# kernel-matrix-benchmarks/kernel-matrix-benchmarks

Measured on AMD Instinct MI355X. Metric: point-pair interactions/s (N*M/s) + max |err| vs scipy, D=3 Gaussian, higher is better.
Workload: dtype f32

## Files before the change

### kernel_matrix_benchmarks_amd/csrc/kmvp_api.hip

```cpp
#include "kmvp_ctx.hpp"

namespace kmvp {

Rccl g_rccl;

namespace {
thread_local std::string g_create_error;
}

int fail(kmvp_ctx* c, int code, const std::string& msg) {
  if (c) c->err = msg;
  else g_create_error = msg;
  return code;
}
const char* create_error() { return g_create_error.c_str(); }

int ensure(kmvp_ctx* c, DevBuf& b, size_t bytes) {
  if (bytes <= b.cap && b.p) return KMVP_OK;
  if (b.p) {
    HIP_TRY(c, hipFree(b.p));
    b.p = nullptr;
    b.cap = 0;
  }
  if (bytes == 0) bytes = 16;
// ... 38 lines not shown
  kmvp_ctx* c = new kmvp_ctx();
  c->device = device;
  bool ok = hipSetDevice(device) == hipSuccess &&
            hipStreamCreateWithFlags(&c->stream, hipStreamNonBlocking) == hipSuccess;
  for (int i = 0; ok && i < 5; ++i) ok = hipEventCreate(&c->ev[i]) == hipSuccess;
  if (!ok) {
    fail(nullptr, KMVP_E_DEVICE, "cannot create stream/events on the device");
    if (status) *status = KMVP_E_DEVICE;
    kmvp_destroy(c);
    return nullptr;
  }
  if (status) *status = KMVP_OK;
  return c;
}

void kmvp_destroy(kmvp_ctx* c) {
  if (!c) return;
  (void)hipSetDevice(c->device);
  if (c->stream) (void)hipStreamSynchronize(c->stream);
  if (c->comm && g_rccl.CommDestroy) g_rccl.CommDestroy(c->comm);
  for (DevBuf* b : {&c->y_raw, &c->x_raw, &c->b_raw, &c->xs, &c->rec, &c->x_scaled, &c->y_scaled,
                    &c->part, &c->partd, &c->aux, &c->sortbuf, &c->perm, &c->sums, &c->out, &c->scratch, &c->sdiag, &c->precond, &c->knn, &c->xchg, &c->kexp, &c->kshift, &c->xchgk, &c->kflag,
                    &c->sk_xs_x, &c->sk_rec_y, &c->sk_xs_y, &c->sk_rec_x, &c->sk_state, &c->km_xs, &c->km_rec, &c->km_part, &c->km_state, &c->ms_xs, &c->ms_state, &c->ms_tmp,
                    &c->cell_tperm, &c->cell_sperm, &c->cell_tgrp, &c->cell_sgrp, &c->cell_slot, &c->cell_tmeta, &c->cell_sums, &c->cell_skey, &c->cell_scentre, &c->cell_scale})
    release(*b);
  for (int i = 0; i < 5; ++i)
    if (c->ev[i]) (void)hipEventDestroy(c->ev[i]);
  if (c->stream) (void)hipStreamDestroy(c->stream);
  delete c;
}

const char* kmvp_last_error(const kmvp_ctx* c) { return c ? c->err.c_str() : create_error(); }

int kmvp_set_points(kmvp_ctx* c, const void* y, int64_t M, const void* x_or_null, int64_t N, int D,
                    int dtype, int64_t j_offset, int64_t M_total) {
  if (!c) return KMVP_E_INVALID;
  if (dtype != KMVP_F32 && dtype != KMVP_F64 && dtype != KMVP_BF16)
    return fail(c, KMVP_E_INVALID, "unknown dtype");
  if (M < 0 || N < 0 || D < 1) return fail(c, KMVP_E_INVALID, "bad shape");
  if ((M > 0 && !y) || (N > 0 && !x_or_null && N != M))
    return fail(c, KMVP_E_INVALID, "same_points (x == NULL) needs N == M");
  if (M_total < M || j_offset < 0 || j_offset + M > M_total)
    return fail(c, KMVP_E_INVALID, "shard [j_offset, j_offset+M) is outside [0, M_total)");
  HIP_TRY(c, hipSetDevice(c->device));
  const size_t es = elem_size(dtype);
  int rc;
  if ((rc = ensure(c, c->y_raw, (size_t)M * D * es))) return rc;
// ... 274 lines not shown

int kmvp_set_option(kmvp_ctx* c, const char* key, int64_t value) {
  if (!c || !key) return KMVP_E_INVALID;
  const std::string k(key);
  if (k == "feed") {
    if (value < -1 || value > 1) return fail(c, KMVP_E_INVALID, "feed must be -1 (auto), 0 or 1");
    c->opt_feed = (int)value;
  } else if (k == "targets_per_lane") {
    if (value != 0 && value != 1 && value != 2 && value != 4 && value != 8)
      return fail(c, KMVP_E_INVALID, "targets_per_lane must be 0 (auto), 1, 2, 4 or 8");
    c->opt_T = (int)value;
  } else if (k == "segments") {
    if (value < 0 || value > 65535) return fail(c, KMVP_E_INVALID, "segments out of range");
    c->opt_segments = (int)value;
  } else if (k == "fast_sqdists") {
    if (value < -1 || value > 4) return fail(c, KMVP_E_INVALID, "fast_sqdists must be -1 (auto), 0, 1, 2, 3 or 4");
    c->opt_fast = (int)value;
  } else if (k == "cellmm_shape") {
    if (value < -1 || value > 1) return fail(c, KMVP_E_INVALID, "cellmm_shape must be -1 (by size), 0 (32x32x16) or 1 (16x16x32)");
    c->opt_cellmm_shape = (int)value;
  } else if (k == "cell_fused") {
    if (value < -1 || value > 1) return fail(c, KMVP_E_INVALID, "cell_fused must be -1 (automatic), 0 (two launches) or 1 (one launch where it applies)");
    c->opt_cell_fused = (int)value;
  } else if (k == "cell_shared_build") {
    if (value < -1 || value > 1) return fail(c, KMVP_E_INVALID, "cell_shared_build must be -1 (automatic), 0 (never) or 1 (wherever a workgroup is one-cell)");
    c->opt_cell_shared_build = (int)value;
  } else if (k == "mfma_variant") {
    if (value != -1 && value != 0 && value != 1 && value != 4 && value != 5)
      return fail(c, KMVP_E_INVALID, "mfma_variant must be -1 (by kernel), 0, 1, 4 or 5");
    c->opt_mfma_variant = (int)value;
  } else if (k == "same_points_global") {
    c->opt_same_global = value != 0;
  } else if (k == "partial_shard") {
    c->opt_partial = value != 0;
  } else if (k == "fast_tiles") {
    if (value != 0 && value != 1 && value != 2 && value != 4 && value != 8)
      return fail(c, KMVP_E_INVALID, "fast_tiles must be 0 (auto), 1, 2, 4 or 8");
    c->opt_fast_tiles = (int)value;
  } else if (k == "meanshift_compact") {
    if (value < -1 || value > 1) return fail(c, KMVP_E_INVALID, "meanshift_compact must be -1 (default), 0 or 1");
    c->opt_meanshift_compact = (int)value;
  } else if (k == "chunk") {
    if (value < 8 || value > (1 << 24)) return fail(c, KMVP_E_INVALID, "chunk out of range");
    c->opt_chunk = (int)value;
  } else {
    return fail(c, KMVP_E_INVALID, "unknown option " + k);
  }
  return KMVP_OK;
}

int64_t kmvp_device_bytes(const kmvp_ctx* c) {
  if (!c) return 0;
  size_t t = 0;
  for (const DevBuf* b : {&c->y_raw, &c->x_raw, &c->b_raw, &c->xs, &c->rec, &c->x_scaled,
                          &c->y_scaled, &c->part, &c->partd, &c->aux, &c->sortbuf, &c->perm, &c->sums, &c->out, &c->scratch, &c->sdiag, &c->precond, &c->knn, &c->xchg, &c->kexp, &c->kshift, &c->xchgk, &c->kflag,
                    &c->sk_xs_x, &c->sk_rec_y, &c->sk_xs_y, &c->sk_rec_x, &c->sk_state, &c->km_xs, &c->km_rec, &c->km_part, &c->km_state, &c->ms_xs, &c->ms_state, &c->ms_tmp,
                          &c->cell_tperm, &c->cell_sperm, &c->cell_tgrp, &c->cell_sgrp, &c->cell_slot, &c->cell_tmeta, &c->cell_sums, &c->cell_skey, &c->cell_scentre, &c->cell_scale})
    t += b->cap;
  return (int64_t)t;
}
double kmvp_last_kernel_ms(const kmvp_ctx* c) { return c ? c->last_kernel_ms : 0.0; }
double kmvp_last_total_ms(const kmvp_ctx* c) { return c ? c->last_total_ms : 0.0; }
double kmvp_last_allreduce_ms(const kmvp_ctx* c) { return c ? c->last_allreduce_ms : 0.0; }
const char* kmvp_last_kernel_name(const kmvp_ctx* c) { return c ? c->last_kernel_name : ""; }
const char* kmvp_last_dispatch_note(const kmvp_ctx* c) { return c ? c->note.c_str() : ""; }

}
```

### kernel_matrix_benchmarks_amd/csrc/kmvp_cell.hpp

```cpp
#pragma once
#include <hip/hip_runtime.h>
#include <stdint.h>

#include "kmvp_fast.hpp"

namespace kmvp {

constexpr int CELL_STAGE_TILES = 4;
constexpr int CELL_A_BYTES = CELL_TILE * 32;
constexpr int CELL_TILE_BYTES = CELL_A_BYTES + CELL_TILE * 16;
constexpr int CELL_HDR_OFF = CELL_STAGE_TILES * CELL_TILE_BYTES;
constexpr int CELL_STAGE_BYTES = 8192;
static_assert(CELL_HDR_OFF + CELL_STAGE_TILES * 16 <= CELL_STAGE_BYTES, "stage image too small");
constexpr float CELL_T_MAX = 0.016f;
constexpr int CELL_MAX_GRID = 1024;

struct CellGrid {
  float lo[3];
  float h[3], inv_h[3];
  int g[3];
};

__host__ __device__ inline float cell_centre(unsigned key, int a, const CellGrid& grid) {
  return grid.lo[a] + ((float)((key >> (10 * a)) & 1023u) + 0.5f) * grid.h[a];
}

struct CellArgs {
  const float* xd;
  const float* tmeta;
  const unsigned char* img;
  double* part;
  int64_t n_slots;
  int64_t tile_base;
  int64_t m_stages;
  int64_t seg_stages;
  int segments;
  int tile_blocks;
  int chunk_stages;
};

template <int SIG, int TT>
__global__ void __launch_bounds__(BLOCK_THREADS) cell_kernel(const CellArgs a) {
  constexpr int NE = (SIG == SIG_NORM) ? 2 : 1;
  constexpr int SB = CELL_STAGE_BYTES;
  constexpr int PIECES = SB / (16 * BLOCK_THREADS);
  constexpr float LOG2E = 1.4426950408889634f;
// ... 180 lines not shown
```

### kernel_matrix_benchmarks_amd/csrc/kmvp_cell_pack.hpp

```cpp
#pragma once
#include "kmvp_cell.hpp"

namespace kmvp {

__global__ void cell_keys_kernel(const float* __restrict__ p, int64_t n, int D, CellGrid grid,
                                 unsigned* __restrict__ keys, int* __restrict__ vals) {
  const int64_t i = (int64_t)blockIdx.x * blockDim.x + threadIdx.x;
  if (i >= n) return;
  unsigned key = 0;
  for (int a = 0; a < D; ++a) {
    int c = (int)floorf((p[i * D + a] - grid.lo[a]) * grid.inv_h[a]);
    c = c < 0 ? 0 : (c >= grid.g[a] ? grid.g[a] - 1 : c);
    key |= (unsigned)c << (10 * a);
  }
  keys[i] = key;
  vals[i] = (int)i;
}

__global__ void __launch_bounds__(CELL_TILE) pack_cell_targets_kernel(
    const float* __restrict__ x, const int* __restrict__ perm, const int* __restrict__ gstart,
    const int* __restrict__ gcnt, const unsigned* __restrict__ gkey, int64_t n_groups, int D, CellGrid grid,
    float* __restrict__ xd, float* __restrict__ tmeta, int* __restrict__ slot_of) {
  const int64_t g = blockIdx.x;
  const int r = threadIdx.x;
  const int64_t gg = g < n_groups ? g : n_groups - 1;
  const unsigned key = gkey[gg];
  const bool valid = g < n_groups && r < gcnt[g];
  const int64_t idx = valid ? perm[gstart[g] + r] : 0;
  float d[4] = {0.f, 0.f, 0.f, 0.f}, c[3] = {0.f, 0.f, 0.f};
  for (int a = 0; a < D; ++a) {
    c[a] = cell_centre(key, a, grid);
    d[a] = valid ? x[idx * D + a] - c[a] : 0.f;
  }
  *reinterpret_cast<f32x4*>(xd + (g * CELL_TILE + r) * 4) = f32x4{d[0], d[1], d[2], 0.f};
  const bool empty = g >= n_groups || gcnt[g] == 0;
  if (r == 0)
    *reinterpret_cast<f32x4*>(tmeta + g * 4) = f32x4{c[0], c[1], c[2], __builtin_bit_cast(float, key | (empty ? 1u << 30 : 0u))};
  if (valid) slot_of[idx] = (int)(g * CELL_TILE + r);
// ... 62 lines not shown
```

### kernel_matrix_benchmarks_amd/csrc/kmvp_cellmm_pack.hpp

```cpp
#pragma once
#include "kmvp_cellmm.hpp"

namespace kmvp {

__global__ void __launch_bounds__(CELL_TILE) pack_cellmm_points_kernel(
    const float* __restrict__ y, const int* __restrict__ perm, const int* __restrict__ gstart,
    const int* __restrict__ gcnt, const unsigned* __restrict__ gkey, int64_t n_groups, int D, CellGrid grid,
    unsigned char* __restrict__ img) {
  const int64_t g = blockIdx.x;
  const int r = threadIdx.x;
  unsigned char* stage = img + (g / CMM_STAGE_TILES) * CMM_STAGE_BYTES;
  const int q = (int)(g % CMM_STAGE_TILES);
  const bool real_tile = g < n_groups;
  const unsigned key = real_tile ? gkey[g] : 0u;
  const bool valid = real_tile && r < gcnt[g];
  const int64_t idx = valid ? perm[gstart[g] + r] : 0;
  float e[3] = {0.f, 0.f, 0.f}, c[3] = {0.f, 0.f, 0.f};
  for (int a = 0; a < D; ++a) {
    c[a] = cell_centre(key, a, grid);
    e[a] = valid ? y[idx * D + a] - c[a] : 0.f;
  }
  const float e2 = e[0] * e[0] + e[1] * e[1] + e[2] * e[2];
  *reinterpret_cast<f32x4*>(stage + CMM_E_OFF + (q * CELL_TILE + r) * 16) =
      f32x4{2.f * e[0], 2.f * e[1], 2.f * e[2], e2 * -1.4426950408889634f};
  if (r == 0)
    *reinterpret_cast<f32x4*>(stage + CMM_HDR_OFF + q * 16) =
        f32x4{c[0], c[1], c[2], __int_as_float(real_tile ? (int)key : -1)};
}

__global__ void cellmm_absmax_kernel(const float* __restrict__ b, int64_t n, int E, int col, unsigned* __restrict__ out) {
  unsigned m = 0;
  for (int64_t i = (int64_t)blockIdx.x * blockDim.x + threadIdx.x; i < n; i += (int64_t)gridDim.x * blockDim.x) {
    const unsigned v = (unsigned)__float_as_int(b[i * E + col]) & 0x7fffffffu;
    m = v > m ? v : m;
  }
  for (int off = 32; off > 0; off >>= 1) {
    const unsigned o = (unsigned)__shfl_xor((int)m, off);
    m = o > m ? o : m;
  }
  if ((threadIdx.x & 63) == 0 && m) atomicMax(out, m);
}

__global__ void cellmm_scale_kernel(const unsigned* __restrict__ bmax_bits, int wlog2, int density,
                                    float* __restrict__ scale) {
  float bmax = density ? 1.f : __int_as_float((int)*bmax_bits);
  int ex = 0;
  if (bmax > 0.f && bmax < INFINITY) {
    int eb;
    (void)frexpf(bmax * 0.104f, &eb);
    ex = 15 - eb - wlog2;
    ex = ex < -100 ? -100 : (ex > 100 ? 100 : ex);
  }
  scale[0] = ldexpf(1.f, ex);
  scale[1] = ldexpf(1.f, -ex - 6);
}

__global__ void __launch_bounds__(CELL_TILE) pack_cellmm_signal_kernel(
    const float* __restrict__ b, int E, int col, const int* __restrict__ perm, const int* __restrict__ gstart,
    const int* __restrict__ gcnt, int64_t n_groups, const float* __restrict__ scale, unsigned char* __restrict__ img) {
  const int64_t g = blockIdx.x;
  const int r = threadIdx.x;
  unsigned char* stage = img + (g / CMM_STAGE_TILES) * CMM_STAGE_BYTES;
  const int q = (int)(g % CMM_STAGE_TILES);
  const bool valid = g < n_groups && r < gcnt[g];
  const float bj = valid ? (b ? b[(int64_t)perm[gstart[g] + r] * E + col] : 1.f) : 0.f;
  *reinterpret_cast<float*>(stage + CMM_B_OFF + (q * CELL_TILE + r) * 4) = bj * scale[0];
}

}
```

### kernel_matrix_benchmarks_amd/csrc/kmvp_ctx.hpp

```cpp
#pragma once
#include <dlfcn.h>
#include <hip/hip_runtime.h>
#include <rccl/rccl.h>
#include <stdint.h>
#include <stdlib.h>
#include <string.h>

#include <algorithm>
#include <cmath>
#include <string>
#include <vector>

#include "../../include/kmvp.h"
#include "kmvp_internal.hpp"

namespace kmvp {

enum : int { LAYOUT_LOWD = 0, LAYOUT_FAST = 1, LAYOUT_MFMA = 2, LAYOUT_CFAST = 3, LAYOUT_CELL = 4, LAYOUT_CELL64 = 5, LAYOUT_CELLMM = 6, LAYOUT_FASTMM = 7, LAYOUT_CFASTMM = 8 };

struct DevBuf {
  void* p = nullptr;
  size_t cap = 0;
};

// ... 60 lines not shown
  using DevBuf = kmvp::DevBuf;
  int device = 0;
  hipStream_t stream = nullptr;
  hipEvent_t ev[5] = {nullptr, nullptr, nullptr, nullptr, nullptr};
  std::string err;

  int dtype = -1;
  int D = 0, E = 0;
  int64_t M = 0, N = 0, j_offset = 0, m_total = 0;
  bool same_points = false;
  bool have_points = false, have_signal = false, density = false;
  bool async_product = false;
  bool diag_on = false;
  int64_t diag_n = 0;
  double diag_ridge = 0.0, diag_min = 0.0;

  DevBuf y_raw, x_raw, b_raw;
  DevBuf xs, rec;
  DevBuf partd;
  DevBuf aux;
  DevBuf sortbuf, perm;
  DevBuf x_scaled, y_scaled;
  DevBuf cell_tperm, cell_sperm, cell_tgrp, cell_sgrp, cell_slot, cell_tmeta, cell_sums, cell_skey, cell_scentre, cell_scale;
  DevBuf part, sums, out;
  DevBuf xchg;
  DevBuf kexp, kshift, xchgk;
  DevBuf kflag;
  DevBuf scratch;
  DevBuf knn;
  DevBuf sdiag;
  DevBuf precond;
  int precond_rank = 0;
  int pc_built = 0;
  int pc_used = 0;
  int pc_kernel = -1, pc_rank = 0;
  uint64_t pc_points_ver = 0, pc_diag_ver = 0;
  uint64_t diag_ver = 0;
  float last_precond_ms = 0.f;
  double pc_logdet_c = 0.0;
  DevBuf sk_xs_x, sk_rec_y, sk_xs_y, sk_rec_x, sk_state;
  uint64_t sk_points_ver = 0;
  DevBuf km_xs, km_rec, km_part, km_state;
  uint64_t km_points_ver = 0;
  DevBuf ms_xs, ms_state, ms_tmp;
  uint64_t points_ver = 0, signal_ver = 0;
  int packed_layout = -1;
  int packed_kernel = -1, packed_sig = -1, packed_T = -1;
  uint64_t packed_points_ver = 0, packed_signal_ver = 0;
  int gen_kernel = -1;
  uint64_t gen_points_ver = 0;
  int64_t out_n = 0;
  int out_e = 0;

  int opt_feed = -1, opt_T = 0, opt_segments = 0, opt_chunk = 512;
  int opt_fast = -1, opt_fast_tiles = 0;
  int opt_cellmm_shape = -1;
  int opt_cell_shared_build = -1;
  int opt_cell_fused = -1;
  int opt_mfma_variant = -1;
  int opt_meanshift_compact = -1;
  int opt_same_global = 0;
  int opt_partial = 0;
  uint64_t perm_ver = 0;
  uint64_t cell_ver = 0;
  int cell_state = 0;
  int cell_tt = 0, cell_tt_req = 0;
  float cell_lo[3] = {0.f, 0.f, 0.f}, cell_hh[3] = {1.f, 1.f, 1.f};
  int cell_g[3] = {1, 1, 1};
  int64_t cell_n_tiles = 0, cell_m_tiles = 0;
  int64_t cell_n_main = 0, cell_n_rest = 0;
  float cloud_radius2 = INFINITY;
  uint64_t centre_ver = 0;

  ncclComm_t comm = nullptr;
  int rank = 0, world = 1;
  kmvp_host_allreduce_fn host_xchg = nullptr;
  void* host_user = nullptr;
  std::vector<double> host_buf;
  bool exchanges() const { return comm != nullptr || host_xchg != nullptr; }

  int comm_count = 1;
  float last_kernel_ms = 0.f, last_total_ms = 0.f, last_allreduce_ms = 0.f;
  const char* last_kernel_name = "";
  std::string note;
};

namespace kmvp {

// ... 83 lines not shown
```

### kernel_matrix_benchmarks_amd/csrc/kmvp_plan.hpp

```cpp
#pragma once
#include <algorithm>
#include <cstdint>
#include <vector>

namespace kmvp {

constexpr int WAVES_PER_BLOCK = 4;
constexpr int CELL_TILE = 32;
constexpr int CELL_REST_TT = 2;
constexpr int STAGED_TILE = 32;
constexpr int64_t SMALL_PROBLEM_TARGETS = 32768;
constexpr int SEG_SPLIT_FROM = 16;
constexpr int64_t MAX_GRID = 0x7fffffff;

inline int64_t round_up(int64_t v, int64_t q) { return (v + q - 1) / q * q; }
inline bool small_problem(int64_t N) { return N < SMALL_PROBLEM_TARGETS; }


struct SegmentRule {
  int64_t stage_bytes;
  int cols;
  int64_t min_seg = 1;
  bool small = false;
  int64_t l2_seg_bytes = 2 << 20;
// ... 191 lines not shown
  g.main_grid = s.grid(0);
  g.rest_grid = s.grid(1);
  g.total = g.main_grid + g.rest_grid;
  g.fused = opt_fused != 0 && tt > CELL_REST_TT && s.blocks[1] > 0 && g.total <= MAX_GRID;
  return g;
}


constexpr int CELL_SHARED_TT = 8;

constexpr bool cell_shared_build(int tt, int opt) { return opt != 0 && tt >= CELL_SHARED_TT; }

inline int64_t count_one_cell_blocks(const unsigned* keys, int64_t n_main, int tt) {
  const int64_t per_block = (int64_t)tt * WAVES_PER_BLOCK;
  int64_t one = 0;
  for (int64_t t = 0; t + per_block <= n_main; t += per_block) {
    bool same = true;
    for (int w = 1; w < WAVES_PER_BLOCK; ++w) same = same && keys[t + (int64_t)w * tt] == keys[t];
    one += same ? 1 : 0;
  }
  return one;
}

}
```

### kernel_matrix_benchmarks_amd/csrc/kmvp_product.hip

```cpp
#include "kmvp_ctx.hpp"
#include <vector>
#include "kmvp_cell_pack.hpp"
#include "kmvp_cell64_pack.hpp"
#include "kmvp_cellmm_pack.hpp"
#include "kmvp_cfast_pack.hpp"
#include "kmvp_fast_pack.hpp"
#include "kmvp_fastmm_pack.hpp"
#include "kmvp_cfastmm_pack.hpp"
#include "kmvp_mfma_pack.hpp"

namespace kmvp {
namespace {

template <typename real>
hipError_t launch_lowd(int kernel, int D, int E, int sig, LowdTuning tune,
                       const LowdArgs<real>& args, dim3 grid, hipStream_t s, const char** name);
template <>
hipError_t launch_lowd<float>(int kernel, int D, int E, int sig, LowdTuning tune,
                              const LowdArgs<float>& args, dim3 grid, hipStream_t s,
                              const char** name) {
  switch (kernel) {
    case K_GAUSSIAN: return launch_lowd_gaussian_f32(D, E, sig, tune, args, grid, s, name);
    case K_ABSEXP: return launch_lowd_absexp_f32(D, E, sig, tune, args, grid, s, name);
    case K_INVDIST: return launch_lowd_invdist_f32(D, E, sig, tune, args, grid, s, name);
// ... 1109 lines not shown
  a.scale = scale;
  a.m_total = c->m_total;
  const dim3 grid((unsigned)p.grid);
  const int64_t pieces = m_stages * (CF_GROUP / 32) * (MODE ? 2 : 1) * 2 * 64;
  return run_column_blocks(
      c, key, sig, p, cb, false, online ? "cfastmm_kernel with the per-target online shift (targets != sources)" : nullptr,
      [&](int col0, int nb) {
        hipLaunchKernelGGL(pack_cfastmm_signal_kernel, dim3(blocks_for(pieces)), dim3(256), 0, c->stream,
                           (const float*)c->b_raw.p, (const float*)cb.sigma, (const int*)c->perm.p, (unsigned char*)c->rec.p,
                           M, m_stages, E, col0, nb, MODE);
      },
      [&](int nb) {
        a.NE = nb;
        a.part = (double*)c->part.p;
        hipError_t le = launch_cfastmm(kernel, MODE, TT, online, a, grid, c->stream, &c->last_kernel_name);
        if (le == hipErrorInvalidValue) return fail(c, KMVP_E_UNSUPPORTED, "no cfastmm_kernel for this kernel / tile count");
        HIP_TRY(c, le);
        return (int)KMVP_OK;
      });
}


int cell_sort(kmvp_ctx* c, const void* pts, int64_t n, const CellGrid& grid, kmvp_ctx::DevBuf& perm,
              std::vector<unsigned>& keys, kmvp_ctx::DevBuf* keys_dev = nullptr) {
  int rc;
  const int D = c->D;
  const size_t keys_bytes = (size_t)n * sizeof(unsigned);
  SortBufs b;
  if ((rc = sort_buffers(c, n, b))) return rc;
  if ((rc = ensure(c, perm, (size_t)n * sizeof(int)))) return rc;
  if (c->dtype == KMVP_F64)
    hipLaunchKernelGGL(cell64_keys_kernel, dim3(blocks_for(n)), dim3(256), 0, c->stream, (const double*)pts, n, D, grid,
                       b.keys_in, b.vals_in);
  else
    hipLaunchKernelGGL(cell_keys_kernel, dim3(blocks_for(n)), dim3(256), 0, c->stream, (const float*)pts, n, D, grid,
                       b.keys_in, b.vals_in);
  HIP_TRY(c, hipGetLastError());
  HIP_TRY(c, sort_pairs_u32(b.tmp, &b.tmp_bytes, b.keys_in, b.keys_out, b.vals_in, (int*)perm.p, n, c->stream));
  keys.resize((size_t)n);
  HIP_TRY(c, hipMemcpyAsync(keys.data(), b.keys_out, keys_bytes, hipMemcpyDeviceToHost, c->stream));
  if (keys_dev) {
    if ((rc = ensure(c, *keys_dev, keys_bytes))) return rc;
    HIP_TRY(c, hipMemcpyAsync(keys_dev->p, b.keys_out, keys_bytes, hipMemcpyDeviceToDevice, c->stream));
  }
  HIP_TRY(c, hipStreamSynchronize(c->stream));
  return KMVP_OK;
}

int upload_tiles(kmvp_ctx* c, const TileList& l, kmvp_ctx::DevBuf& grp) {
  const size_t G = l.size();
  int rc;
  if ((rc = ensure(c, grp, 3 * std::max<size_t>(G, 1) * sizeof(int)))) return rc;
  HIP_TRY(c, hipMemcpyAsync(grp.p, l.start.data(), G * sizeof(int), hipMemcpyHostToDevice, c->stream));
  HIP_TRY(c, hipMemcpyAsync((int*)grp.p + G, l.count.data(), G * sizeof(int), hipMemcpyHostToDevice, c->stream));
  HIP_TRY(c, hipMemcpyAsync((int*)grp.p + 2 * G, l.key.data(), G * sizeof(int), hipMemcpyHostToDevice, c->stream));
  HIP_TRY(c, hipStreamSynchronize(c->stream));
// ... 14 lines not shown
    if (!(cells <= CELL_MAX_GRID)) return false;
    grid.g[a] = (int)cells;
    if (half > 0.f) {
      grid.h[a] = (float)(2.0 * half / cells);
      grid.inv_h[a] = 1.f / grid.h[a];
    }
  }
  return true;
}
void cell_store_grid(kmvp_ctx* c, const CellGrid& grid) {
  for (int a = 0; a < 3; ++a) {
    c->cell_lo[a] = grid.lo[a];
    c->cell_g[a] = grid.g[a];
    c->cell_hh[a] = grid.h[a];
  }
}
void cell_load_grid(const kmvp_ctx* c, CellGrid& grid) {
  for (int a = 0; a < 3; ++a) {
    grid.lo[a] = c->cell_lo[a];
    grid.g[a] = c->cell_g[a];
    grid.h[a] = c->cell_hh[a];
    grid.inv_h[a] = 1.f / c->cell_hh[a];
  }
}

inline double cell_ps_per_tile(int TT) { return TT >= 8 ? CMM_PS_PER_TILE_MAIN : (TT >= 4 ? CMM_PS_PER_TILE_TT4 : CMM_PS_PER_TILE_REST); }

int cell_prepare(kmvp_ctx* c, int TT) {
  if (c->cell_ver == c->points_ver && c->cell_state != 0 && (c->cell_state < 0 || c->cell_tt_req == TT)) return KMVP_OK;
  c->cell_tt_req = TT;
  c->cell_ver = c->points_ver;
  c->cell_state = -1;
  const int D = c->D;
  if (D > CELL_MAX_D || !(c->cloud_radius2 < INFINITY) || c->N > 0x3fffffff || c->M > 0x3fffffff) return KMVP_OK;
  float aux[FAST_AUX_FLOATS];
  HIP_TRY(c, hipMemcpyAsync(aux, c->aux.p, sizeof(aux), hipMemcpyDeviceToHost, c->stream));
  HIP_TRY(c, hipStreamSynchronize(c->stream));
  CellGrid grid;
  if (!cell_make_grid(aux, D, (float)(std::sqrt(2.f * CELL_T_MAX / (float)D)), grid)) return KMVP_OK;
  int rc;
  std::vector<unsigned> keys;
  if ((rc = cell_sort(c, c->y_raw.p, c->M, grid, c->cell_sperm, keys))) return rc;
  const TileList sources = cell_tiles(keys.data(), c->M);
  if ((rc = upload_tiles(c, sources, c->cell_sgrp))) return rc;
  c->cell_m_tiles = (int64_t)sources.size();
  if (!c->same_points && (rc = cell_sort(c, c->x_raw.p, c->N, grid, c->cell_tperm, keys))) return rc;
  if (TT == 0) {
    double best = INFINITY;
    for (int t : {8, 4, 2}) {
      int64_t nm, nr;
      cell_split_count(keys.data(), (int64_t)keys.size(), t, &nm, &nr);
      const double cost = cell_ps_per_tile(t) * (double)nm + cell_ps_per_tile(2) * (double)nr;
      if (cost < best) {
        best = cost;
        TT = t;
      }
    }
  }
  if ((rc = upload_tiles(c, cell_tiles_split(keys.data(), (int64_t)keys.size(), TT, &c->cell_n_main, &c->cell_n_rest), c->cell_tgrp)))
    return rc;
  c->cell_n_tiles = c->cell_n_main + c->cell_n_rest;
  c->cell_tt = TT;
  cell_store_grid(c, grid);
  c->cell_state = 1;
  c->packed_layout = -1;
  return KMVP_OK;
}

double cell_padding(const kmvp_ctx* c) {
  const double t = (double)c->cell_n_tiles * CELL_TILE / (double)std::max<int64_t>(c->N, 1);
  const double s = (double)c->cell_m_tiles * CELL_TILE / (double)std::max<int64_t>(c->M, 1);
  return std::max(t, s);
}

CellSplit cell_plan(const kmvp_ctx* c, int stage_tiles, SegmentRule main) {
  return cell_split(c->N, c->cell_m_tiles, c->cell_n_main, c->cell_n_rest, c->cell_tt, c->opt_segments, stage_tiles, main);
}
double* cell_region(const kmvp_ctx* c, const CellSplit& s, int cols, int r) { return (double*)c->part.p + s.region_offset(cols, r); }
template <class Args>
void cell_args(const kmvp_ctx* c, const CellSplit& s, int cols, int r, Args& a) {
  a.part = cell_region(c, s, cols, r);
  a.n_slots = s.slots[r];
  a.tile_base = r ? c->cell_n_main : 0;
  a.seg_stages = s.seg_stages[r];
  a.segments = s.segments[r];
  a.tile_blocks = (int)s.blocks[r];
}
inline int cell_tt(const kmvp_ctx* c, int r) { return r ? CELL_REST_TT : c->cell_tt; }

int pack_cell_targets(kmvp_ctx* c, const CellGrid& grid) {
  const int64_t n_tiles = c->cell_n_tiles;
  const float* x_raw = (const float*)(c->same_points ? c->y_raw.p : c->x_raw.p);
  const int* tperm = (const int*)(c->same_points ? c->cell_sperm.p : c->cell_tperm.p);
  const int* tgrp = (const int*)c->cell_tgrp.p;
  int rc;
  if ((rc = ensure(c, c->xs, (size_t)n_tiles * CELL_TILE * 4 * sizeof(float)))) return rc;
  if ((rc = ensure(c, c->cell_tmeta, (size_t)n_tiles * 4 * sizeof(float)))) return rc;
  if ((rc = ensure(c, c->cell_slot, (size_t)c->N * sizeof(int)))) return rc;
  hipLaunchKernelGGL(pack_cell_targets_kernel, dim3((unsigned)n_tiles), dim3(CELL_TILE), 0, c->stream, x_raw, tperm,
                     tgrp, tgrp + n_tiles, (const unsigned*)(tgrp + 2 * n_tiles), n_tiles, c->D,
                     grid, (float*)c->xs.p, (float*)c->cell_tmeta.p, (int*)c->cell_slot.p);
  return KMVP_OK;
}


int run_product_cell(kmvp_ctx* c, int sig) {
  const int D = c->D;
  const int E = 1;
  const int NE = sig == SIG_NORM ? 2 : 1;
  const int64_t N = c->N;
  SegmentRule rule(CELL_STAGE_BYTES, NE);
  rule.min_seg = 4;
  const CellSplit s = cell_plan(c, CELL_STAGE_TILES, rule);
  const int64_t m_stages = s.m_stages, n_slots = s.n_slots;
  int rc;
  CellGrid grid;
  cell_load_grid(c, grid);

  const PackKey key = {LAYOUT_CELL, K_GAUSSIAN, c->cell_tt};
  const int* sgrp = (const int*)c->cell_sgrp.p;
  if (points_stale(c, key) && (rc = pack_cell_targets(c, grid))) return rc;
  if (signal_stale(c, key, sig)) {
    if ((rc = ensure(c, c->rec, (size_t)m_stages * CELL_STAGE_BYTES))) return rc;
    hipLaunchKernelGGL(pack_cell_sources_kernel, dim3((unsigned)(m_stages * CELL_STAGE_TILES)), dim3(CELL_TILE), 0,
                       c->stream, (const float*)c->y_raw.p,
                       sig == SIG_DENSITY ? (const float*)nullptr : (const float*)c->b_raw.p,
                       (const int*)c->cell_sperm.p, sgrp, sgrp + c->cell_m_tiles,
                       (const unsigned*)(sgrp + 2 * c->cell_m_tiles), c->cell_m_tiles, D, grid,
                       (unsigned char*)c->rec.p);
  }
  HIP_TRY(c, hipGetLastError());
  record_packed(c, key, sig);

  if ((rc = ensure(c, c->part, s.part_doubles(NE) * sizeof(double)))) return rc;
  CellArgs a;
  a.xd = (const float*)c->xs.p;
  a.tmeta = (const float*)c->cell_tmeta.p;
  a.img = (const unsigned char*)c->rec.p;
  a.m_stages = m_stages;
  a.chunk_stages = std::max(1, c->opt_chunk / (CELL_TILE * CELL_STAGE_TILES));
  HIP_TRY(c, mark(c, 0));
  hipError_t le = hipSuccess;
  for (int r = 0; r < 2 && le == hipSuccess; ++r)
    if (s.blocks[r] > 0) {
      cell_args(c, s, NE, r, a);
      le = launch_cell_gaussian(sig, cell_tt(c, r), a, dim3((unsigned)s.grid(r)), c->stream, &c->last_kernel_name);
    }
  if (le == hipErrorInvalidValue) return fail(c, KMVP_E_UNSUPPORTED, "fast_tiles must be 1, 2, 4 or 8");
  HIP_TRY(c, le);
  HIP_TRY(c, mark(c, 1));

  if ((rc = ensure(c, c->sums, (size_t)NE * N * sizeof(double)))) return rc;
  if ((rc = ensure(c, c->cell_sums, (size_t)NE * n_slots * sizeof(double)))) return rc;
  for (int r = 0; r < 2; ++r)
    if (s.blocks[r] > 0)
      hipLaunchKernelGGL(reduce_region_kernel, dim3(blocks_for((int64_t)NE * s.slots[r])), dim3(256), 0, c->stream,
                         (const double*)cell_region(c, s, NE, r), (double*)c->cell_sums.p, s.slots[r], NE, s.segments[r], n_slots,
                         r ? s.slots[0] : (int64_t)0);
  hipLaunchKernelGGL(gather_cells_kernel, dim3(blocks_for((int64_t)NE * N)), dim3(256), 0, c->stream,
                     (const double*)c->cell_sums.p, (const int*)c->cell_slot.p, (double*)c->sums.p, N, n_slots, NE);
  HIP_TRY(c, hipGetLastError());
  return finish_product(c, (int64_t)NE * N, N, N, E, sig);
}


int cellmm_wlog2(const kmvp_ctx* c) {
  double arg = 0.0;
  for (int a = 0; a < c->D; ++a) arg += (double)c->cell_hh[a] * ((double)c->cell_g[a] * c->cell_hh[a]);
  return (int)std::ceil(arg * 1.4426950408889634);
}

int run_product_cellmm(kmvp_ctx* c, int sig) {
  const int D = c->D;
  const int E = sig == SIG_DENSITY ? 1 : c->E;
  const int NE = sig == SIG_NORM ? E + 1 : E;
  const int64_t N = c->N;
  const int TT = c->cell_tt;
  SegmentRule rule(CMM_STAGE_BYTES, 1);
  rule.min_seg = 2;
  rule.l2_seg_bytes = 3 << 20;
  rule.target_blocks = 7168;
  const CellSplit s = cell_plan(c, CMM_STAGE_TILES, rule);
  const int64_t m_stages = s.m_stages, n_slots = s.n_slots;
  int rc;
  CellGrid grid;
  cell_load_grid(c, grid);

  const PackKey key = {LAYOUT_CELLMM, K_GAUSSIAN, TT};
  const int image_sig = NE > 1 ? -1 : sig;
  const bool sig_stale = signal_stale(c, key, image_sig);
  const int* sgrp = (const int*)c->cell_sgrp.p;
  if ((rc = ensure(c, c->cell_scale, 64))) return rc;
  float* scale = (float*)c->cell_scale.p;
  unsigned* bmax = (unsigned*)c->cell_scale.p + 4;
  HIP_TRY(c, mark(c, 0));
  if (points_stale(c, key)) {
    if ((rc = pack_cell_targets(c, grid))) return rc;
    if ((rc = ensure(c, c->rec, (size_t)m_stages * CMM_STAGE_BYTES))) return rc;
    hipLaunchKernelGGL(pack_cellmm_points_kernel, dim3((unsigned)(m_stages * CMM_STAGE_TILES)), dim3(CELL_TILE), 0,
                       c->stream, (const float*)c->y_raw.p, (const int*)c->cell_sperm.p, sgrp, sgrp + c->cell_m_tiles,
                       (const unsigned*)(sgrp + 2 * c->cell_m_tiles), c->cell_m_tiles, D, grid, (unsigned char*)c->rec.p);
    HIP_TRY(c, hipGetLastError());
  }
  record_packed(c, key, image_sig);

  if ((rc = ensure(c, c->part, s.part_doubles(1) * sizeof(double)))) return rc;
  if ((rc = ensure(c, c->sums, (size_t)NE * N * sizeof(double)))) return rc;
  if ((rc = ensure(c, c->cell_sums, (size_t)NE * n_slots * sizeof(double)))) return rc;
  const int shape = c->opt_cellmm_shape >= 0 ? c->opt_cellmm_shape : ((TT >= 8 && c->N >= 500000 && c->M >= 100000) ? 1 : 0);
  FusedCellGrid fg = fused_cell_grid(s, TT, c->opt_cell_fused);
  if (shape != 1) fg.fused = false;
  CellmmArgs a;
  a.xd = (const float*)c->xs.p;
  a.tmeta = (const float*)c->cell_tmeta.p;
  a.img = (const unsigned char*)c->rec.p;
  a.scale = scale;
  a.m_stages = m_stages;
  a.shared_build = cell_shared_build(TT, c->opt_cell_shared_build) ? 1 : 0;
  if (NE == 1 && !sig_stale) HIP_TRY(c, mark(c, 0));
  for (int col = 0; col < NE; ++col) {
    if (sig_stale) {
      const float* b = (sig == SIG_DENSITY || col == E) ? (const float*)nullptr : (const float*)c->b_raw.p;
      HIP_TRY(c, hipMemsetAsync(bmax, 0, sizeof(unsigned), c->stream));
      if (b)
        hipLaunchKernelGGL(cellmm_absmax_kernel, dim3((unsigned)std::min<int64_t>(1024, (c->M + 255) / 256)), dim3(256), 0,
                           c->stream, b, c->M, E, col, bmax);
      hipLaunchKernelGGL(cellmm_scale_kernel, dim3(1), dim3(1), 0, c->stream, (const unsigned*)bmax, cellmm_wlog2(c),
                         b ? 0 : 1, scale);
      hipLaunchKernelGGL(pack_cellmm_signal_kernel, dim3((unsigned)(m_stages * CMM_STAGE_TILES)), dim3(CELL_TILE), 0,
                         c->stream, b, E, col, (const int*)c->cell_sperm.p, sgrp, sgrp + c->cell_m_tiles, c->cell_m_tiles,
                         (const float*)scale, (unsigned char*)c->rec.p);
      HIP_TRY(c, hipGetLastError());
      if (NE == 1) HIP_TRY(c, mark(c, 0));
    }
    hipError_t le = hipSuccess;
    if (fg.fused) {
      CellmmArgs ar = a;
      cell_args(c, s, 1, 0, a);
      cell_args(c, s, 1, 1, ar);
      le = launch_cellmm16_fused(TT, a, ar, fg.main_grid, fg.rest_grid, c->stream, &c->last_kernel_name);
    } else {
      for (int r = 0; r < 2 && le == hipSuccess; ++r)
        if (s.blocks[r] > 0) {
          cell_args(c, s, 1, r, a);
          le = launch_cellmm_gaussian(cell_tt(c, r), shape, a, dim3((unsigned)s.grid(r)), c->stream, &c->last_kernel_name);
        }
    }
    if (le == hipErrorInvalidValue) return fail(c, KMVP_E_UNSUPPORTED, "fast_tiles must be 1, 2, 4 or 8");
    HIP_TRY(c, le);
    if (NE == 1) HIP_TRY(c, mark(c, 1));
    double* col_sums = (double*)c->cell_sums.p + (size_t)col * n_slots;
// ... 419 lines not shown
      c->note.clear();
      const int rc = run_product_cellmm(c, sig);
      if (c->opt_fast < 0) c->note += cost;
      return rc;
    }
  }
  if (f32 && kernel == K_ABSEXP && !c->density && c->D > CFAST_MAX_D && c->D <= FMM_MAX_D && (c->opt_fast < 0 || c->opt_fast == 1)) {
    const bool pays = c->D > LOWD_MAX_D || c->E + (normalise ? 1 : 0) > LOWD_MAX_E;
    if (radius_ok(c, kernel) && (c->opt_fast == 1 || pays)) {
      c->note.clear();
      return run_product_fastmm(c, K_ABSEXP, sig);
    }
  }
  const bool invdist_square = kernel == K_INVDIST && (c->same_points || c->opt_same_global) && c->N == c->m_total;
  if (f32 && (kernel == K_GAUSSIAN || kernel == K_ABSEXP || invdist_square) && !c->density && c->E > 1 && c->D <= CFAST_MAX_D &&
      (c->opt_fast == 2 || (c->opt_fast < 0 && c->E + (normalise ? 1 : 0) >= CFMM_AUTO_MIN_COLS))) {
    c->note.clear();
    return run_product_cfastmm(c, kernel, sig);
  }
  if (f32 && c->D <= FAST_MAX_D && (c->density || c->E == 1)) {
    const bool global_ok = kernel == K_GAUSSIAN && radius_ok(c, kernel);
    const bool centred_ok = c->D <= CFAST_MAX_D && (kernel != K_INVDIST || invdist_square);
    if (cells) {
      c->note.clear();
      if (c->opt_fast != 4 && cellmm_in_range(c))
        return run_product_cellmm(c, sig);
      if (c->opt_fast != 4) c->note = "cell_kernel instead of cellmm_kernel: the clouds are outside the radius rule (f16 operand range)";
      return run_product_cell(c, sig);
    }
    if (c->opt_fast == 1 || (c->opt_fast < 0 && global_ok)) return run_product_fast(c, kernel, sig);
    if (centred_ok && (c->opt_fast == 2 || c->opt_fast < 0)) return run_product_cfast(c, kernel, sig);
  }
  if (c->dtype == KMVP_F64 && kernel == K_GAUSSIAN && c->D <= CELL_MAX_D && (c->density || c->E == 1) &&
      c->centre_ver == c->points_ver && cells64_considered(c)) {
    int rc = cell64_prepare(c);
    if (rc) return rc;
    if (c->cell_state == 1 &&
        (c->opt_fast == 3 || (double)c->cell_n_tiles * CELL64_TILE <= CELL_AUTO_MAX_PAD * (double)c->N))
      return run_product_cell64(c, sig);
  }
  if (c->D <= LOWD_MAX_D && !c->density && c->E > LOWD_MAX_E) {
    if (c->note.empty()) c->note = "E > 4 signal columns: the difference form runs once per block of four columns";
    return c->dtype == KMVP_F64 ? run_product_blocked<double>(c, kernel, sig) : run_product_blocked<float>(c, kernel, sig);
  }
  if (c->dtype == KMVP_F64) return run_product_t<double>(c, kernel, sig);
  return run_product_t<float>(c, kernel, sig);
}


static int run_target_columns(kmvp_ctx* c, int kernel, const std::string& what, bool dscale) {
// ... 289 lines not shown
```

Before: 42480 billion.

## Cut cell columns along z by point count to balance cell tiles

Adds a count-cut cell layout for D=3 f32: points get fine z-quantised keys and each x-y column is split into cells holding full tile quanta, bounded by a z-width cap, with per-cell centres stored in a device table. The goal is fewer partially filled (padded) tiles and better load balance in the cell MFMA kernels, which reduces wasted work on empty tile slots. In exchange, z-widths vary per cell, so the f16 scale factor and exponent bounds are recomputed, and there are extra host-side cell building and centre uploads. Enabled automatically for large N and M.

After: 43660 billion (median of 6 runs). +2.8%, better.

```diff
diff --git a/kernel_matrix_benchmarks_amd/csrc/kmvp_api.hip b/kernel_matrix_benchmarks_amd/csrc/kmvp_api.hip
--- a/kernel_matrix_benchmarks_amd/csrc/kmvp_api.hip
+++ b/kernel_matrix_benchmarks_amd/csrc/kmvp_api.hip
@@ -84,7 +84,7 @@
   for (DevBuf* b : {&c->y_raw, &c->x_raw, &c->b_raw, &c->xs, &c->rec, &c->x_scaled, &c->y_scaled,
                     &c->part, &c->partd, &c->aux, &c->sortbuf, &c->perm, &c->sums, &c->out, &c->scratch, &c->sdiag, &c->precond, &c->knn, &c->xchg, &c->kexp, &c->kshift, &c->xchgk, &c->kflag,
                     &c->sk_xs_x, &c->sk_rec_y, &c->sk_xs_y, &c->sk_rec_x, &c->sk_state, &c->km_xs, &c->km_rec, &c->km_part, &c->km_state, &c->ms_xs, &c->ms_state, &c->ms_tmp,
-                    &c->cell_tperm, &c->cell_sperm, &c->cell_tgrp, &c->cell_sgrp, &c->cell_slot, &c->cell_tmeta, &c->cell_sums, &c->cell_skey, &c->cell_scentre, &c->cell_scale})
+                    &c->cell_tperm, &c->cell_sperm, &c->cell_tgrp, &c->cell_sgrp, &c->cell_slot, &c->cell_tmeta, &c->cell_sums, &c->cell_skey, &c->cell_scentre, &c->cell_scale, &c->cell_tcentre, &c->cell_scentre32})
     release(*b);
   for (int i = 0; i < 5; ++i)
     if (c->ev[i]) (void)hipEventDestroy(c->ev[i]);
@@ -405,6 +405,9 @@
   } else if (k == "cell_fused") {
     if (value < -1 || value > 1) return fail(c, KMVP_E_INVALID, "cell_fused must be -1 (automatic), 0 (two launches) or 1 (one launch where it applies)");
     c->opt_cell_fused = (int)value;
+  } else if (k == "cell_balance") {
+    if (value < -1 || value > 1) return fail(c, KMVP_E_INVALID, "cell_balance must be -1 (automatic), 0 (never) or 1 (wherever count-cut cells apply)");
+    c->opt_cell_balance = (int)value;
   } else if (k == "cell_shared_build") {
     if (value < -1 || value > 1) return fail(c, KMVP_E_INVALID, "cell_shared_build must be -1 (automatic), 0 (never) or 1 (wherever a workgroup is one-cell)");
     c->opt_cell_shared_build = (int)value;
@@ -438,7 +441,7 @@
   for (const DevBuf* b : {&c->y_raw, &c->x_raw, &c->b_raw, &c->xs, &c->rec, &c->x_scaled,
                           &c->y_scaled, &c->part, &c->partd, &c->aux, &c->sortbuf, &c->perm, &c->sums, &c->out, &c->scratch, &c->sdiag, &c->precond, &c->knn, &c->xchg, &c->kexp, &c->kshift, &c->xchgk, &c->kflag,
                     &c->sk_xs_x, &c->sk_rec_y, &c->sk_xs_y, &c->sk_rec_x, &c->sk_state, &c->km_xs, &c->km_rec, &c->km_part, &c->km_state, &c->ms_xs, &c->ms_state, &c->ms_tmp,
-                          &c->cell_tperm, &c->cell_sperm, &c->cell_tgrp, &c->cell_sgrp, &c->cell_slot, &c->cell_tmeta, &c->cell_sums, &c->cell_skey, &c->cell_scentre, &c->cell_scale})
+                          &c->cell_tperm, &c->cell_sperm, &c->cell_tgrp, &c->cell_sgrp, &c->cell_slot, &c->cell_tmeta, &c->cell_sums, &c->cell_skey, &c->cell_scentre, &c->cell_scale, &c->cell_tcentre, &c->cell_scentre32})
     t += b->cap;
   return (int64_t)t;
 }
diff --git a/kernel_matrix_benchmarks_amd/csrc/kmvp_cell.hpp b/kernel_matrix_benchmarks_amd/csrc/kmvp_cell.hpp
--- a/kernel_matrix_benchmarks_amd/csrc/kmvp_cell.hpp
+++ b/kernel_matrix_benchmarks_amd/csrc/kmvp_cell.hpp
@@ -19,9 +19,11 @@
   float lo[3];
   float h[3], inv_h[3];
   int g[3];
+  const float* centres = nullptr;
 };
 
 __host__ __device__ inline float cell_centre(unsigned key, int a, const CellGrid& grid) {
+  if (grid.centres) return grid.centres[4 * (size_t)key + a];
   return grid.lo[a] + ((float)((key >> (10 * a)) & 1023u) + 0.5f) * grid.h[a];
 }
 
diff --git a/kernel_matrix_benchmarks_amd/csrc/kmvp_cell_pack.hpp b/kernel_matrix_benchmarks_amd/csrc/kmvp_cell_pack.hpp
--- a/kernel_matrix_benchmarks_amd/csrc/kmvp_cell_pack.hpp
+++ b/kernel_matrix_benchmarks_amd/csrc/kmvp_cell_pack.hpp
@@ -14,6 +14,22 @@
     key |= (unsigned)c << (10 * a);
   }
   keys[i] = key;
+  vals[i] = (int)i;
+}
+
+__global__ void cell_fine_keys_kernel(const float* __restrict__ p, int64_t n, CellGrid grid, double zq_per_unit,
+                                      unsigned* __restrict__ keys, int* __restrict__ vals) {
+  const int64_t i = (int64_t)blockIdx.x * blockDim.x + threadIdx.x;
+  if (i >= n) return;
+  unsigned column = 0;
+  for (int a = 0; a < 2; ++a) {
+    int c = (int)floorf((p[i * 3 + a] - grid.lo[a]) * grid.inv_h[a]);
+    c = c < 0 ? 0 : (c >= grid.g[a] ? grid.g[a] - 1 : c);
+    column |= (unsigned)c << (10 * a);
+  }
+  int zq = (int)floor(((double)p[i * 3 + 2] - (double)grid.lo[2]) * zq_per_unit);
+  zq = zq < 0 ? 0 : (zq >= CELL_ZQ ? CELL_ZQ - 1 : zq);
+  keys[i] = (column << CELL_ZQ_BITS) | (unsigned)zq;
   vals[i] = (int)i;
 }
 
diff --git a/kernel_matrix_benchmarks_amd/csrc/kmvp_cellmm_pack.hpp b/kernel_matrix_benchmarks_amd/csrc/kmvp_cellmm_pack.hpp
--- a/kernel_matrix_benchmarks_amd/csrc/kmvp_cellmm_pack.hpp
+++ b/kernel_matrix_benchmarks_amd/csrc/kmvp_cellmm_pack.hpp
@@ -41,13 +41,13 @@
   if ((threadIdx.x & 63) == 0 && m) atomicMax(out, m);
 }
 
-__global__ void cellmm_scale_kernel(const unsigned* __restrict__ bmax_bits, int wlog2, int density,
+__global__ void cellmm_scale_kernel(const unsigned* __restrict__ bmax_bits, int wlog2, float fmax, int density,
                                     float* __restrict__ scale) {
   float bmax = density ? 1.f : __int_as_float((int)*bmax_bits);
   int ex = 0;
   if (bmax > 0.f && bmax < INFINITY) {
     int eb;
-    (void)frexpf(bmax * 0.104f, &eb);
+    (void)frexpf(bmax * fmax, &eb);
     ex = 15 - eb - wlog2;
     ex = ex < -100 ? -100 : (ex > 100 ? 100 : ex);
   }
diff --git a/kernel_matrix_benchmarks_amd/csrc/kmvp_ctx.hpp b/kernel_matrix_benchmarks_amd/csrc/kmvp_ctx.hpp
--- a/kernel_matrix_benchmarks_amd/csrc/kmvp_ctx.hpp
+++ b/kernel_matrix_benchmarks_amd/csrc/kmvp_ctx.hpp
@@ -106,6 +106,7 @@
   DevBuf sortbuf, perm;
   DevBuf x_scaled, y_scaled;
   DevBuf cell_tperm, cell_sperm, cell_tgrp, cell_sgrp, cell_slot, cell_tmeta, cell_sums, cell_skey, cell_scentre, cell_scale;
+  DevBuf cell_tcentre, cell_scentre32;
   DevBuf part, sums, out;
   DevBuf xchg;
   DevBuf kexp, kshift, xchgk;
@@ -140,6 +141,7 @@
   int opt_fast = -1, opt_fast_tiles = 0;
   int opt_cellmm_shape = -1;
   int opt_cell_shared_build = -1;
+  int opt_cell_balance = -1;
   int opt_cell_fused = -1;
   int opt_mfma_variant = -1;
   int opt_meanshift_compact = -1;
@@ -148,6 +150,9 @@
   uint64_t perm_ver = 0;
   uint64_t cell_ver = 0;
   int cell_state = 0;
+  int cell_balance_req = -1;
+  bool cell_balanced = false;
+  float cell_zw = 0.f;
   int cell_tt = 0, cell_tt_req = 0;
   float cell_lo[3] = {0.f, 0.f, 0.f}, cell_hh[3] = {1.f, 1.f, 1.f};
   int cell_g[3] = {1, 1, 1};
diff --git a/kernel_matrix_benchmarks_amd/csrc/kmvp_plan.hpp b/kernel_matrix_benchmarks_amd/csrc/kmvp_plan.hpp
--- a/kernel_matrix_benchmarks_amd/csrc/kmvp_plan.hpp
+++ b/kernel_matrix_benchmarks_amd/csrc/kmvp_plan.hpp
@@ -237,4 +237,74 @@
   return one;
 }
 
-}
+
+constexpr int CELL_ZQ_BITS = 12;
+constexpr int CELL_ZQ = 1 << CELL_ZQ_BITS;
+constexpr int CELL_BALANCE_MIN_CAP = 16;
+
+struct CountCell {
+  int64_t first, count;
+  int zlo, zhi;
+  unsigned column;
+};
+
+inline std::vector<CountCell> count_cut_cells(const unsigned* fine, int64_t n, int cap, int64_t quantum, int64_t full) {
+  std::vector<CountCell> cells;
+  cells.reserve((size_t)(n / std::max<int64_t>(full, 1)) + 16);
+  const unsigned zmask = (unsigned)CELL_ZQ - 1u;
+  for (int64_t p = 0; p < n;) {
+    const unsigned column = fine[p] >> CELL_ZQ_BITS;
+    const int zlo = (int)(fine[p] & zmask);
+    int64_t e = p + 1;
+    while (e < n && e - p < full && (fine[e] >> CELL_ZQ_BITS) == column && (int)(fine[e] & zmask) - zlo < cap) ++e;
+    const bool by_cap = e < n && e - p < full && (fine[e] >> CELL_ZQ_BITS) == column;
+    int64_t count = e - p;
+    if (by_cap && count >= quantum) count = count / quantum * quantum;
+    cells.push_back({p, count, zlo, (int)(fine[p + count - 1] & zmask), column});
+    p += count;
+  }
+  return cells;
+}
+
+inline float count_cell_zcentre(double lo, double bw, int zlo, int zhi) { return (float)(lo + 0.5 * (double)(zlo + zhi + 1) * bw); }
+
+inline TileList count_cell_source_tiles(const std::vector<CountCell>& cells, int tile = CELL_TILE) {
+  TileList l;
+  l.reserve(cells.size() * 33 + 16);
+  for (size_t i = 0; i < cells.size(); ++i) {
+    const CountCell& c = cells[i];
+    l.add_cell(c.first, c.first, c.first + c.count, (unsigned)i, (c.count + tile - 1) / tile, 0, tile);
+  }
+  return l;
+}
+
+inline TileList count_cell_target_tiles(const std::vector<CountCell>& cells, int TT, int64_t* n_main, int64_t* n_rest) {
+  TileList main, rest;
+  main.reserve(cells.size() * 33 + 64);
+  const int64_t per_block = (int64_t)TT * WAVES_PER_BLOCK;
+  for (int pass = 0; pass < 2; ++pass)
+    for (size_t i = 0; i < cells.size(); ++i) {
+      const CountCell& c = cells[i];
+      const CellTiles s = split_cell_tiles((c.count + CELL_TILE - 1) / CELL_TILE, TT);
+      const int64_t m = s.main_live + s.main_empty;
+      if ((m > 0 && m % per_block == 0) != (pass == 0)) continue;
+      main.add_cell(c.first, c.first, c.first + c.count, (unsigned)i, s.main_live, s.main_empty, CELL_TILE);
+      rest.add_cell(c.first, c.first + s.main_live * CELL_TILE, c.first + c.count, (unsigned)i, s.rest_live, s.rest_empty, CELL_TILE);
+    }
+  main.pad_to((size_t)per_block);
+  rest.pad_to((size_t)CELL_REST_TT * WAVES_PER_BLOCK);
+  *n_main = (int64_t)main.size();
+  *n_rest = (int64_t)rest.size();
+  main.append(rest);
+  return main;
+}
+
+constexpr bool cell_balance_applies(int D, bool f32, int tt, int cap) {
+  return D == 3 && f32 && tt == CELL_SHARED_TT && cap >= CELL_BALANCE_MIN_CAP;
+}
+constexpr int64_t CELLMM16_AUTO_N = 500000, CELLMM16_AUTO_M = 100000;
+constexpr bool cell_balance_taken(int opt, bool applies, int64_t N, int64_t M) {
+  return opt != 0 && applies && (opt > 0 || (N >= CELLMM16_AUTO_N && M >= CELLMM16_AUTO_M));
+}
+
+}
diff --git a/kernel_matrix_benchmarks_amd/csrc/kmvp_product.hip b/kernel_matrix_benchmarks_amd/csrc/kmvp_product.hip
--- a/kernel_matrix_benchmarks_amd/csrc/kmvp_product.hip
+++ b/kernel_matrix_benchmarks_amd/csrc/kmvp_product.hip
@@ -1155,7 +1155,7 @@
 
 
 int cell_sort(kmvp_ctx* c, const void* pts, int64_t n, const CellGrid& grid, kmvp_ctx::DevBuf& perm,
-              std::vector<unsigned>& keys, kmvp_ctx::DevBuf* keys_dev = nullptr) {
+              std::vector<unsigned>& keys, kmvp_ctx::DevBuf* keys_dev = nullptr, double zq_per_unit = 0.0) {
   int rc;
   const int D = c->D;
   const size_t keys_bytes = (size_t)n * sizeof(unsigned);
@@ -1165,6 +1165,9 @@
   if (c->dtype == KMVP_F64)
     hipLaunchKernelGGL(cell64_keys_kernel, dim3(blocks_for(n)), dim3(256), 0, c->stream, (const double*)pts, n, D, grid,
                        b.keys_in, b.vals_in);
+  else if (zq_per_unit > 0.0)
+    hipLaunchKernelGGL(cell_fine_keys_kernel, dim3(blocks_for(n)), dim3(256), 0, c->stream, (const float*)pts, n, grid,
+                       zq_per_unit, b.keys_in, b.vals_in);
   else
     hipLaunchKernelGGL(cell_keys_kernel, dim3(blocks_for(n)), dim3(256), 0, c->stream, (const float*)pts, n, D, grid,
                        b.keys_in, b.vals_in);
@@ -1225,13 +1228,66 @@
     grid.h[a] = c->cell_hh[a];
     grid.inv_h[a] = 1.f / c->cell_hh[a];
   }
+  grid.centres = nullptr;
+}
+CellGrid cell_side_grid(const kmvp_ctx* c, CellGrid grid, bool targets) {
+  if (c->cell_balanced) grid.centres = (const float*)((targets && !c->same_points) ? c->cell_tcentre.p : c->cell_scentre32.p);
+  return grid;
+}
+
+
+constexpr float CELL_Z_WIDTH_MAX = 0.125f;
+constexpr float CMM_F_LATTICE = 0.104f;
+int cell_balance_cap(const CellGrid& grid, double* zq_per_unit, double* bucket) {
+  const double room = 2.0 * CELL_T_MAX - (double)grid.h[0] * grid.h[0] - (double)grid.h[1] * grid.h[1];
+  const double extent = (double)grid.g[2] * grid.h[2];
+  *bucket = extent / CELL_ZQ;
+  *zq_per_unit = CELL_ZQ / extent;
+  if (!(room > 0.0) || !(extent > 0.0)) return 0;
+  const double width = std::min(std::sqrt(room), (double)CELL_Z_WIDTH_MAX);
+  return (int)std::min<double>(CELL_ZQ, std::floor(width / *bucket));
+}
+
+int upload_cell_centres(kmvp_ctx* c, const CellGrid& grid, double bucket, const std::vector<CountCell>& cells, kmvp_ctx::DevBuf& buf) {
+  std::vector<float> tab(4 * std::max<size_t>(cells.size(), 1), 0.f);
+  for (size_t i = 0; i < cells.size(); ++i) {
+    tab[4 * i + 0] = cell_centre(cells[i].column, 0, grid);
+    tab[4 * i + 1] = cell_centre(cells[i].column, 1, grid);
+    tab[4 * i + 2] = count_cell_zcentre(grid.lo[2], bucket, cells[i].zlo, cells[i].zhi);
+  }
+  int rc;
+  if ((rc = ensure(c, buf, tab.size() * sizeof(float)))) return rc;
+  HIP_TRY(c, hipMemcpyAsync(buf.p, tab.data(), tab.size() * sizeof(float), hipMemcpyHostToDevice, c->stream));
+  HIP_TRY(c, hipStreamSynchronize(c->stream));
+  return KMVP_OK;
+}
+
+int cell_prepare_balanced(kmvp_ctx* c, const CellGrid& grid, int TT, int cap, double zq_per_unit, double bucket) {
+  const int64_t quantum = (int64_t)CELL_TILE * TT, full = quantum * WAVES_PER_BLOCK;
+  int rc;
+  std::vector<unsigned> keys;
+  if ((rc = cell_sort(c, c->y_raw.p, c->M, grid, c->cell_sperm, keys, nullptr, zq_per_unit))) return rc;
+  std::vector<CountCell> cells = count_cut_cells(keys.data(), c->M, cap, c->same_points ? quantum : (int64_t)CELL_TILE, full);
+  const TileList sources = count_cell_source_tiles(cells);
+  if ((rc = upload_tiles(c, sources, c->cell_sgrp))) return rc;
+  c->cell_m_tiles = (int64_t)sources.size();
+  if ((rc = upload_cell_centres(c, grid, bucket, cells, c->cell_scentre32))) return rc;
+  if (!c->same_points) {
+    if ((rc = cell_sort(c, c->x_raw.p, c->N, grid, c->cell_tperm, keys, nullptr, zq_per_unit))) return rc;
+    cells = count_cut_cells(keys.data(), c->N, cap, quantum, full);
+    if ((rc = upload_cell_centres(c, grid, bucket, cells, c->cell_tcentre))) return rc;
+  }
+  return upload_tiles(c, count_cell_target_tiles(cells, TT, &c->cell_n_main, &c->cell_n_rest), c->cell_tgrp);
 }
 
 inline double cell_ps_per_tile(int TT) { return TT >= 8 ? CMM_PS_PER_TILE_MAIN : (TT >= 4 ? CMM_PS_PER_TILE_TT4 : CMM_PS_PER_TILE_REST); }
 
 int cell_prepare(kmvp_ctx* c, int TT) {
-  if (c->cell_ver == c->points_ver && c->cell_state != 0 && (c->cell_state < 0 || c->cell_tt_req == TT)) return KMVP_OK;
+  if (c->cell_ver == c->points_ver && c->cell_state != 0 && c->cell_balance_req == c->opt_cell_balance &&
+      (c->cell_state < 0 || c->cell_tt_req == TT))
+    return KMVP_OK;
   c->cell_tt_req = TT;
+  c->cell_balance_req = c->opt_cell_balance;
   c->cell_ver = c->points_ver;
   c->cell_state = -1;
   const int D = c->D;
@@ -1260,7 +1316,14 @@
       }
     }
   }
-  if ((rc = upload_tiles(c, cell_tiles_split(keys.data(), (int64_t)keys.size(), TT, &c->cell_n_main, &c->cell_n_rest), c->cell_tgrp)))
+  double zq_per_unit, bucket;
+  const int cap = cell_balance_cap(grid, &zq_per_unit, &bucket);
+  c->cell_balanced = false;
+  if (cell_balance_taken(c->opt_cell_balance, cell_balance_applies(D, c->dtype == KMVP_F32, TT, cap), c->N, c->M)) {
+    c->cell_balanced = true;
+    c->cell_zw = (float)((double)cap * bucket);
+    if ((rc = cell_prepare_balanced(c, grid, TT, cap, zq_per_unit, bucket))) return rc;
+  } else if ((rc = upload_tiles(c, cell_tiles_split(keys.data(), (int64_t)keys.size(), TT, &c->cell_n_main, &c->cell_n_rest), c->cell_tgrp)))
     return rc;
   c->cell_n_tiles = c->cell_n_main + c->cell_n_rest;
   c->cell_tt = TT;
@@ -1302,7 +1365,7 @@
   if ((rc = ensure(c, c->cell_slot, (size_t)c->N * sizeof(int)))) return rc;
   hipLaunchKernelGGL(pack_cell_targets_kernel, dim3((unsigned)n_tiles), dim3(CELL_TILE), 0, c->stream, x_raw, tperm,
                      tgrp, tgrp + n_tiles, (const unsigned*)(tgrp + 2 * n_tiles), n_tiles, c->D,
-                     grid, (float*)c->xs.p, (float*)c->cell_tmeta.p, (int*)c->cell_slot.p);
+                     cell_side_grid(c, grid, true), (float*)c->xs.p, (float*)c->cell_tmeta.p, (int*)c->cell_slot.p);
   return KMVP_OK;
 }
 
@@ -1329,7 +1392,7 @@
                        c->stream, (const float*)c->y_raw.p,
                        sig == SIG_DENSITY ? (const float*)nullptr : (const float*)c->b_raw.p,
                        (const int*)c->cell_sperm.p, sgrp, sgrp + c->cell_m_tiles,
-                       (const unsigned*)(sgrp + 2 * c->cell_m_tiles), c->cell_m_tiles, D, grid,
+                       (const unsigned*)(sgrp + 2 * c->cell_m_tiles), c->cell_m_tiles, D, cell_side_grid(c, grid, false),
                        (unsigned char*)c->rec.p);
   }
   HIP_TRY(c, hipGetLastError());
@@ -1369,9 +1432,13 @@
 
 int cellmm_wlog2(const kmvp_ctx* c) {
   double arg = 0.0;
-  for (int a = 0; a < c->D; ++a) arg += (double)c->cell_hh[a] * ((double)c->cell_g[a] * c->cell_hh[a]);
+  for (int a = 0; a < c->D; ++a) {
+    const double w = (c->cell_balanced && a == 2) ? (double)c->cell_zw : (double)c->cell_hh[a];
+    arg += w * ((double)c->cell_g[a] * c->cell_hh[a]);
+  }
   return (int)std::ceil(arg * 1.4426950408889634);
 }
+float cellmm_fmax(const kmvp_ctx* c) { return c->cell_balanced ? std::max(CMM_F_LATTICE, c->cell_zw) : CMM_F_LATTICE; }
 
 int run_product_cellmm(kmvp_ctx* c, int sig) {
   const int D = c->D;
@@ -1402,7 +1469,8 @@
     if ((rc = ensure(c, c->rec, (size_t)m_stages * CMM_STAGE_BYTES))) return rc;
     hipLaunchKernelGGL(pack_cellmm_points_kernel, dim3((unsigned)(m_stages * CMM_STAGE_TILES)), dim3(CELL_TILE), 0,
                        c->stream, (const float*)c->y_raw.p, (const int*)c->cell_sperm.p, sgrp, sgrp + c->cell_m_tiles,
-                       (const unsigned*)(sgrp + 2 * c->cell_m_tiles), c->cell_m_tiles, D, grid, (unsigned char*)c->rec.p);
+                       (const unsigned*)(sgrp + 2 * c->cell_m_tiles), c->cell_m_tiles, D, cell_side_grid(c, grid, false),
+                       (unsigned char*)c->rec.p);
     HIP_TRY(c, hipGetLastError());
   }
   record_packed(c, key, image_sig);
@@ -1410,7 +1478,7 @@
   if ((rc = ensure(c, c->part, s.part_doubles(1) * sizeof(double)))) return rc;
   if ((rc = ensure(c, c->sums, (size_t)NE * N * sizeof(double)))) return rc;
   if ((rc = ensure(c, c->cell_sums, (size_t)NE * n_slots * sizeof(double)))) return rc;
-  const int shape = c->opt_cellmm_shape >= 0 ? c->opt_cellmm_shape : ((TT >= 8 && c->N >= 500000 && c->M >= 100000) ? 1 : 0);
+  const int shape = c->opt_cellmm_shape >= 0 ? c->opt_cellmm_shape : ((TT >= 8 && c->N >= CELLMM16_AUTO_N && c->M >= CELLMM16_AUTO_M) ? 1 : 0);
   FusedCellGrid fg = fused_cell_grid(s, TT, c->opt_cell_fused);
   if (shape != 1) fg.fused = false;
   CellmmArgs a;
@@ -1429,7 +1497,7 @@
         hipLaunchKernelGGL(cellmm_absmax_kernel, dim3((unsigned)std::min<int64_t>(1024, (c->M + 255) / 256)), dim3(256), 0,
                            c->stream, b, c->M, E, col, bmax);
       hipLaunchKernelGGL(cellmm_scale_kernel, dim3(1), dim3(1), 0, c->stream, (const unsigned*)bmax, cellmm_wlog2(c),
-                         b ? 0 : 1, scale);
+                         cellmm_fmax(c), b ? 0 : 1, scale);
       hipLaunchKernelGGL(pack_cellmm_signal_kernel, dim3((unsigned)(m_stages * CMM_STAGE_TILES)), dim3(CELL_TILE), 0,
                          c->stream, b, E, col, (const int*)c->cell_sperm.p, sgrp, sgrp + c->cell_m_tiles, c->cell_m_tiles,
                          (const float*)scale, (unsigned char*)c->rec.p);
@@ -1895,10 +1963,12 @@
     const bool global_ok = kernel == K_GAUSSIAN && radius_ok(c, kernel);
     const bool centred_ok = c->D <= CFAST_MAX_D && (kernel != K_INVDIST || invdist_square);
     if (cells) {
-      c->note.clear();
+      c->note = c->cell_balanced ? "count-cut cells: the lattice's columns cut along z by point count (cell_balance)" : "";
       if (c->opt_fast != 4 && cellmm_in_range(c))
         return run_product_cellmm(c, sig);
-      if (c->opt_fast != 4) c->note = "cell_kernel instead of cellmm_kernel: the clouds are outside the radius rule (f16 operand range)";
+      if (c->opt_fast != 4)
+        c->note = std::string(c->note.empty() ? "" : c->note + "; ") +
+                  "cell_kernel instead of cellmm_kernel: the clouds are outside the radius rule (f16 operand range)";
       return run_product_cell(c, sig);
     }
     if (c->opt_fast == 1 || (c->opt_fast < 0 && global_ok)) return run_product_fast(c, kernel, sig);
```
